# ymartin101/RTS

Measured on AMD Instinct MI355X. Metric: Mrays/s (primary+bounces) & ms/pulse, 100k-tri scene, higher is better.
Workload: dtype f64

## Files before the change

### rts_amd/csrc/rts_api.hip

```cpp
#include <cmath>
#include <cstdarg>
#include <cstdio>
#include <cstring>
#include <cstdlib>
#include <dlfcn.h>
#include <algorithm>
#include <chrono>
#include <map>
#include <memory>
#include <mutex>
#include <stdexcept>
#include <string>
#include <thread>
#include "rts_internal.h"
#include "rts_raygen.h"
#include <atomic>

static thread_local char g_err[1024] = "";
void rts_set_error(const char* fmt, ...) { va_list ap; va_start(ap, fmt); vsnprintf(g_err, sizeof(g_err), fmt, ap); va_end(ap); }
extern "C" const char* rts_last_error(void) { return g_err; }
#include "rts_build_id.h"
extern "C" const char* rts_build_id(void) { return RTS_SOURCE_HASH; }

#include <dirent.h>
#include <sched.h>
extern "C" int rts_bind_host_to_device(int device, int* numa_node)
{
    if (numa_node) *numa_node = -1;
    char bdf[64] = {0};
    if (hipDeviceGetPCIBusId(bdf, (int)sizeof(bdf), device) != hipSuccess) { (void)hipGetLastError(); rts_set_error("rts_bind_host_to_device: no PCI address for device %d", device); return RTS_ERR_INVALID; }
    for (char* q = bdf; *q; q++) *q = (char)tolower((unsigned char)*q);
    char path[256]; snprintf(path, sizeof(path), "/sys/bus/pci/devices/%s/numa_node", bdf);
    int node = -1;
    if (FILE* f = fopen(path, "r")) { if (fscanf(f, "%d", &node) != 1) node = -1; fclose(f); }
    if (node < 0) return RTS_OK;
    snprintf(path, sizeof(path), "/sys/devices/system/node/node%d/cpulist", node);
    cpu_set_t want; CPU_ZERO(&want); int n_want = 0;
    if (FILE* f = fopen(path, "r")) {
        int a = 0, b = 0; char sep = 0;
        while (fscanf(f, "%d", &a) == 1) {
            b = a;
            int ch = fgetc(f);
            if (ch == '-') { if (fscanf(f, "%d", &b) != 1) b = a; ch = fgetc(f); }
            for (int k = a; k <= b && k < CPU_SETSIZE; k++) { CPU_SET(k, &want); n_want++; }
            sep = (char)ch; if (sep != ',') break;
        }
        fclose(f);
    }
    if (n_want == 0) return RTS_OK;
    cpu_set_t have; CPU_ZERO(&have);
    if (sched_getaffinity(0, sizeof(have), &have) != 0) return RTS_OK;
    cpu_set_t both; CPU_AND(&both, &want, &have);
    if (CPU_COUNT(&both) == 0) return RTS_OK;
    if (DIR* d = opendir("/proc/self/task")) {
        while (struct dirent* e = readdir(d)) { const int tid = atoi(e->d_name); if (tid > 0) (void)sched_setaffinity(tid, sizeof(both), &both); }
        closedir(d);
    } else (void)sched_setaffinity(0, sizeof(both), &both);
    if (numa_node) *numa_node = node;
    return RTS_OK;
}

extern int rts_fill_i32(hipStream_t st, int32_t* p, int32_t v, size_t n);

__global__ void k_children_to_prims(RtsNode4* __restrict__ nodes, uint32_t n, const uint32_t* __restrict__ leaf_prim)
{
    const uint32_t i = blockIdx.x * blockDim.x + threadIdx.x;
    if (i >= n) return;
    for (int k = 0; k < 4; k++) { const int32_t ch = nodes[i].child[k]; nodes[i].pad[k] = ch; if (ch < 0) nodes[i].child[k] = ~(int32_t)leaf_prim[~ch]; }
}

__global__ void k_node_versions(const RtsNode4* __restrict__ nodes, uint32_t n, RtsNode4* __restrict__ out, int key_mode)
{
    const uint32_t g = blockIdx.x * blockDim.x + threadIdx.x;
    if (g >= n * 8u) return;
    const uint32_t i = g >> 3, o = g & 7u;
    const RtsNode4 nd = nodes[i];
    const bool mx = (o & 1u) != 0u, my = (o & 2u) != 0u, mz = (o & 4u) != 0u;
    float key[4]; int ord[4];
    for (int k = 0; k < 4; k++) {
        const float ex = mx ? -nd.hix[k] : nd.lox[k], ey = my ? -nd.hiy[k] : nd.loy[k], ez = mz ? -nd.hiz[k] : nd.loz[k];
        const float cx = 0.5f * (nd.lox[k] + nd.hix[k]), cy = 0.5f * (nd.loy[k] + nd.hiy[k]), cz = 0.5f * (nd.loz[k] + nd.hiz[k]);
        const float kc = key_mode == 1 ? ((mx ? -cx : cx) + (my ? -cy : cy) + (mz ? -cz : cz)) : (ex + ey + ez);
        key[k] = nd.child[k] == 0x7fffffff ? __builtin_inff() : kc;
        ord[k] = k;
    }
    for (int a = 1; a < 4; a++)
        for (int b = a; b > 0 && key[ord[b]] < key[ord[b - 1]]; b--) { const int t = ord[b]; ord[b] = ord[b - 1]; ord[b - 1] = t; }
    RtsNode4 v;
    for (int j = 0; j < 4; j++) {
        const int k = ord[j];
        v.lox[j] = mx ? nd.hix[k] : nd.lox[k]; v.hix[j] = mx ? nd.lox[k] : nd.hix[k];
        v.loy[j] = my ? nd.hiy[k] : nd.loy[k]; v.hiy[j] = my ? nd.loy[k] : nd.hiy[k];
        v.loz[j] = mz ? nd.hiz[k] : nd.loz[k]; v.hiz[j] = mz ? nd.loz[k] : nd.hiz[k];
        const int32_t ch = nd.child[k];
        v.child[j] = (ch >= 0 && ch != 0x7fffffff) ? (int32_t)(((uint32_t)ch << 3) | o) : ch;
        v.pad[j] = nd.pad[k];
    }
    out[g] = v;
// ... 157 lines not shown
        const RtsMesh& m = meshes[t];
        if ((m.n_triangles && !m.triangles) || (m.n_vertices && !m.vertices) || (m.n_normals && !m.normals)) { rts_set_error("rts_set_scene: target %u has null arrays", t); return RTS_ERR_INVALID; }
        mh[t].n_tris = m.n_triangles; mh[t].n_verts = m.n_vertices; mh[t].n_normals = m.n_normals;
        mh[t].tri_base = (uint32_t)nt; mh[t].vert_base = (uint32_t)nv; mh[t].normal_base = (uint32_t)nn;
        mh[t].refl_coeff = m.refl_coeff; mh[t].refr_index = m.refr_index;
        mh[t].perface = m.n_normals > m.n_vertices;
        nt += m.n_triangles; nv += m.n_vertices; nn += m.n_normals;
        if (nt > 0x7ffffff0ULL || nv > 0x7ffffff0ULL || nn > 0x7ffffff0ULL) { rts_set_error("rts_set_scene: scene too large"); return RTS_ERR_UNSUPPORTED; }
    }
    std::vector<uint32_t> vidx(3*nt), nidx(3*nt), vtarg(nv), ntarg(nn), ptarg(nt);
    std::vector<double> verts(3*nv), normals(3*nn);
    for (uint32_t t = 0; t < n_targets; t++) {
        const RtsMesh& m = meshes[t]; const RtsMeshHost& h = mh[t];
        for (uint32_t i = 0; i < m.n_triangles; i++) {
            for (int k = 0; k < 3; k++) {
                uint32_t v = m.triangles[3*(size_t)i + k];
                if (v >= m.n_vertices) { rts_set_error("rts_set_scene: target %u triangle %u references vertex %u >= %u", t, i, v, m.n_vertices); return RTS_ERR_INVALID; }
                vidx[3*((size_t)h.tri_base + i) + k] = h.vert_base + v;
                uint32_t ni = h.perface ? i : v;
                if (m.n_normals == 0) ni = 0; else if (ni >= m.n_normals) { rts_set_error("rts_set_scene: target %u normal index %u >= %u", t, ni, m.n_normals); return RTS_ERR_INVALID; }
                nidx[3*((size_t)h.tri_base + i) + k] = h.normal_base + ni;
            }
            ptarg[(size_t)h.tri_base + i] = t;
        }
        if (m.n_triangles && m.n_normals == 0 && c->params.interpolate_smooth) { rts_set_error("rts_set_scene: target %u has no normals but interpolate_smooth is set", t); return RTS_ERR_INVALID; }
        for (uint32_t i = 0; i < m.n_vertices; i++) { vtarg[(size_t)h.vert_base + i] = t; for (int k = 0; k < 3; k++) verts[3*((size_t)h.vert_base + i) + k] = m.vertices[3*(size_t)i + k]; }
        for (uint32_t i = 0; i < m.n_normals; i++) { ntarg[(size_t)h.normal_base + i] = t; for (int k = 0; k < 3; k++) normals[3*((size_t)h.normal_base + i) + k] = m.normals[3*(size_t)i + k]; }
    }
    std::unique_ptr<RtsScene> guard(new RtsScene());
    RtsScene* ns = guard.get(); ns->device = c->device;
    RTS_HIP(hipStreamSynchronize(c->stream));
    RTS_HIP(ns->d_tri_vidx.reserve(3*nt + 1)); RTS_HIP(ns->d_tri_nidx.reserve(3*nt + 1)); RTS_HIP(ns->d_vert_targ.reserve(nv + 1)); RTS_HIP(ns->d_norm_targ.reserve(nn + 1));
    RTS_HIP(ns->d_prim_targ.reserve(nt + 1)); RTS_HIP(ns->d_verts_local.reserve(3*nv + 1)); RTS_HIP(ns->d_normals_local.reserve(3*nn + 1));
    if (nt) { RTS_HIP(hipMemcpy(ns->d_tri_vidx.p, vidx.data(), sizeof(uint32_t)*3*nt, hipMemcpyHostToDevice)); RTS_HIP(hipMemcpy(ns->d_tri_nidx.p, nidx.data(), sizeof(uint32_t)*3*nt, hipMemcpyHostToDevice));
              RTS_HIP(hipMemcpy(ns->d_prim_targ.p, ptarg.data(), sizeof(uint32_t)*nt, hipMemcpyHostToDevice)); }
    if (nv) { RTS_HIP(hipMemcpy(ns->d_vert_targ.p, vtarg.data(), sizeof(uint32_t)*nv, hipMemcpyHostToDevice)); RTS_HIP(hipMemcpy(ns->d_verts_local.p, verts.data(), sizeof(double)*3*nv, hipMemcpyHostToDevice)); }
    if (nn) { RTS_HIP(hipMemcpy(ns->d_norm_targ.p, ntarg.data(), sizeof(uint32_t)*nn, hipMemcpyHostToDevice)); RTS_HIP(hipMemcpy(ns->d_normals_local.p, normals.data(), sizeof(double)*3*nn, hipMemcpyHostToDevice)); }
    ns->meshes = mh; ns->n_prims = (uint32_t)nt; ns->n_verts = (uint32_t)nv; ns->n_normals = (uint32_t)nn;

    const auto t_build0 = std::chrono::steady_clock::now();
    RtsSceneTuning st; st.device_build = (c->params.flags & RTS_FLAG_HOST_BUILD) == 0;
    rts_tuning_read(&st, rts_env);
    bool device_build = st.device_build;
    const double split_budget = st.split_budget;
    if (device_build) {
        int rc = rts_lbvh_build_device(c, ns, vidx, mh, st);
        if (rc == RTS_OK && st.fail_device_build) { rts_set_error("rts_set_scene: device builder failure injected (RTS_DEBUG_FAIL_DEVICE_BUILD)"); rc = RTS_ERR_HIP; }
        if (rc != RTS_OK) {
            if (rc == RTS_ERR_INVALID || !st.build_fallback) return rc;
            (void)hipGetLastError();
            fprintf(stderr, "[rts] device hierarchy build failed (%s): falling back to the host builder\n", rts_last_error());
            ns->d_nodes4.release(); ns->d_leaf_prim.release(); ns->blas.clear(); ns->n_nodes = 0; ns->n_leaves = 0;
            device_build = false;
        } else ns->builder = 1;
    }
    if (!device_build) {
        std::vector<RtsNode4> nodes4; std::vector<uint32_t> leaf_prim; std::vector<RtsBlasInfo> blas(n_targets);
        {
            std::vector<std::vector<RtsNode4>> pn(n_targets); std::vector<std::vector<uint32_t>> pl(n_targets); std::vector<int> prc(n_targets, RTS_OK);
            for (uint32_t t0 = 0; t0 < n_targets; t0 += 16) {
                std::vector<std::thread> pool;
                for (uint32_t t = t0; t < std::min(n_targets, t0 + 16); t++)
                    pool.emplace_back([&, t]() { prc[t] = rts_sah_build(meshes[t].vertices, meshes[t].triangles, meshes[t].n_triangles, split_budget, pn[t], pl[t], blas[t]); });
                for (auto& th : pool) th.join();
            }
            for (uint32_t t = 0; t < n_targets; t++) {
                if (prc[t] != RTS_OK) return prc[t];
                const int32_t node_base = (int32_t)nodes4.size(), leaf_base = (int32_t)leaf_prim.size();
                for (RtsNode4 nd : pn[t]) {
                    for (int k = 0; k < 4; k++) { int32_t& ch = nd.child[k]; if (ch == 0x7fffffff) continue; if (ch >= 0) ch += node_base; else ch = ~(~ch + leaf_base); }
                    nodes4.push_back(nd);
                }
                for (uint32_t lp : pl[t]) leaf_prim.push_back(lp + mh[t].tri_base);
                if (blas[t].root >= 0) blas[t].root += node_base;
            }
        }
        RTS_HIP(ns->d_nodes4.reserve(nodes4.size() + 1)); RTS_HIP(ns->d_leaf_prim.reserve(leaf_prim.size() + 1));
        if (!nodes4.empty()) RTS_HIP(hipMemcpy(ns->d_nodes4.p, nodes4.data(), sizeof(RtsNode4)*nodes4.size(), hipMemcpyHostToDevice));
        if (!leaf_prim.empty()) RTS_HIP(hipMemcpy(ns->d_leaf_prim.p, leaf_prim.data(), sizeof(uint32_t)*leaf_prim.size(), hipMemcpyHostToDevice));
        ns->blas = blas; ns->n_nodes = (uint32_t)nodes4.size(); ns->n_leaves = (uint32_t)leaf_prim.size();
        ns->builder = 0;
    }
    if (ns->n_nodes) { k_children_to_prims<<<(ns->n_nodes + 255) / 256, 256, 0, c->stream>>>(ns->d_nodes4.p, ns->n_nodes, ns->d_leaf_prim.p); RTS_HIP(hipGetLastError()); RTS_HIP(hipStreamSynchronize(c->stream)); }
    {
        const bool want = st.node_versions;
        const int key_mode = st.version_key_centre ? 1 : 0;
        size_t free_b = 0, total_b = 0; (void)hipMemGetInfo(&free_b, &total_b);
        const size_t need = (size_t)ns->n_nodes * 8 * sizeof(RtsNode4);
        if (want && ns->n_nodes && ns->n_nodes < (1u << 28) && need < free_b / 4) {
            if (ns->d_nodes4v.reserve((size_t)ns->n_nodes * 8) == hipSuccess) {
                k_node_versions<<<(ns->n_nodes * 8u + 255u) / 256u, 256, 0, c->stream>>>(ns->d_nodes4.p, ns->n_nodes, ns->d_nodes4v.p, key_mode);
                RTS_HIP(hipGetLastError()); RTS_HIP(hipStreamSynchronize(c->stream));
            } else (void)hipGetLastError();
        }
    }
    ns->build_ms = std::chrono::duration<double, std::milli>(std::chrono::steady_clock::now() - t_build0).count();

    rts_scene_unref(c->scene);
    c->scene = guard.release();
    return rts_attach_scene(c);
}

static int rts_attach_scene(RtsContext* c)
{
    const RtsScene* sc = c->scene; const uint32_t n_targets = (uint32_t)sc->meshes.size();
    RTS_HIP(c->d_leaves.reserve((size_t)sc->n_prims + 1));
    RTS_HIP(c->d_verts_world.reserve(3*(size_t)sc->n_verts + 1)); RTS_HIP(c->d_normals_world.reserve(3*(size_t)sc->n_normals + 1));
    {
        const size_t span = offsetof(RtsPinned, cnt);
        RTS_HIP(c->d_params.reserve(span));
        c->p_lc = reinterpret_cast<RtsLaunchConsts*>(c->d_params.p + offsetof(RtsPinned, lc));
        c->p_motion = reinterpret_cast<RtsTargetMotion*>(c->d_params.p + offsetof(RtsPinned, motion));
        c->p_targets = reinterpret_cast<RtsTargetDev*>(c->d_params.p + offsetof(RtsPinned, td));
        c->rcs_uploaded = false;
    }
    c->verts_world_valid = false; c->order_sum_valid = false;
    if (c->hist->refs.load() > 1) { rts_hist_unref(c->hist); c->hist = new RtsTileHist(); }
    c->motion.assign(n_targets, RtsTargetMotion{}); c->motion_valid = false; c->bvh_valid = false; c->hist->n = 0; c->hist->any = false; c->hist->head_hint_valid = false; c->tile_cost_pending = false; c->tile_last_valid = false;
    return RTS_OK;
}

extern "C" int rts_share_scene(RtsHandle dst, RtsHandle src)
{
    if (!dst || !src || dst == src) { rts_set_error("rts_share_scene: needs two distinct handles"); return RTS_ERR_INVALID; }
    if (dst->device != src->device) { rts_set_error("rts_share_scene: handles live on different devices (%d, %d)", dst->device, src->device); return RTS_ERR_INVALID; }
    if (dst->params.interpolate_smooth && !src->params.interpolate_smooth) {
        for (const RtsMeshHost& m : src->scene->meshes) if (m.n_tris && m.n_normals == 0) { rts_set_error("rts_share_scene: the scene has a mesh without normals but the receiving handle interpolates normals"); return RTS_ERR_INVALID; }
    }
    RtsContext* c = dst;
    CHECK_HANDLE(c);
    CHECK_CLOSED(c);
    RTS_HIP(hipStreamSynchronize(c->stream));
    if (dst->scene == src->scene) return RTS_OK;
    rts_scene_unref(dst->scene);
    dst->scene = src->scene; dst->scene->refs++;
    { int rc = rts_attach_scene(dst); if (rc != RTS_OK) return rc; }
    if (dst->tune.share_history && src->tune.share_history && dst->params.width == src->params.width) {
        rts_hist_unref(dst->hist);
        dst->hist = src->hist; dst->hist->refs++;
    }
    return RTS_OK;
}

extern "C" int rts_scene_info(RtsHandle c, RtsSceneInfo* out)
{
    if (!c || !out) { rts_set_error("rts_scene_info: null argument"); return RTS_ERR_INVALID; }
    const RtsScene* sc = c->scene;
    memset(out, 0, sizeof(*out));
    out->n_targets = (uint32_t)sc->meshes.size(); out->n_prims = sc->n_prims; out->n_nodes = sc->n_nodes; out->n_leaves = sc->n_leaves;
    out->handles_sharing = (uint32_t)sc->refs.load(); out->builder = sc->builder; out->build_ms = sc->build_ms;
    out->shared_device_bytes = sc->device_bytes(); out->version_bytes = sc->d_nodes4v.cap * sizeof(RtsNode4);
    out->handle_device_bytes = c->d_leaves.cap * sizeof(RtsLeafTri) + c->d_verts_world.cap * 8 + c->d_normals_world.cap * 8 + c->d_params.cap;
    return RTS_OK;
}

extern "C" int rts_set_receivers(RtsHandle c, const RtsReceiverSphere* rx, uint32_t n_rx)
{
    CHECK_HANDLE(c);
    CHECK_CLOSED(c);
    if (n_rx && !rx) { rts_set_error("rts_set_receivers: null array"); return RTS_ERR_INVALID; }
    if (n_rx > 65535) { rts_set_error("rts_set_receivers: more than 65535 receivers"); return RTS_ERR_UNSUPPORTED; }
    { int rc = check_key_width(c->depth, (uint32_t)c->scene->meshes.size(), n_rx, "rts_set_receivers"); if (rc != RTS_OK) return rc; }
    std::vector<RtsRxDev> h(n_rx);
    for (uint32_t i = 0; i < n_rx; i++) {
        const RtsReceiverSphere& r = rx[i];
        const double vals[8] = { r.centre[0], r.centre[1], r.centre[2], r.radius, r.min_theta, r.max_theta, r.min_phi, r.max_phi };
// ... 1164 lines not shown
```

### rts_amd/csrc/rts_bvh.hip

```cpp
#include <cstring>
#include <hip/hip_runtime.h>
#include "rts_internal.h"
#include "rts_ray_ops.h"

__device__ __forceinline__ void place_one(const double* __restrict__ local, double* __restrict__ world, const uint32_t* __restrict__ targ_of,
                                          const RtsTargetMotion* __restrict__ motion, uint32_t i, bool add_position)
{
    const RtsTargetMotion m = motion[targ_of[i]];
    double x = local[3*i], y = local[3*i+1], z = local[3*i+2];
    if (m.has_rotation) {
        double rx = 0.0, ry = 0.0, rz = 0.0;
        rx += m.rotation[0] * x; rx += m.rotation[1] * y; rx += m.rotation[2] * z;
        ry += m.rotation[3] * x; ry += m.rotation[4] * y; ry += m.rotation[5] * z;
        rz += m.rotation[6] * x; rz += m.rotation[7] * y; rz += m.rotation[8] * z;
        x = rx; y = ry; z = rz;
    }
    if (add_position) { x += m.position[0]; y += m.position[1]; z += m.position[2]; }
    world[3*i] = x; world[3*i+1] = y; world[3*i+2] = z;
}
__global__ void k_place(const double* __restrict__ v_local, double* __restrict__ v_world, const uint32_t* __restrict__ v_targ, uint32_t n_verts,
                        const double* __restrict__ n_local, double* __restrict__ n_world, const uint32_t* __restrict__ n_targ, uint32_t n_normals,
                        const RtsTargetMotion* __restrict__ motion)
{
    const uint32_t i = blockIdx.x * blockDim.x + threadIdx.x;
    if (i < n_verts) place_one(v_local, v_world, v_targ, motion, i, true);
    else if (i - n_verts < n_normals) place_one(n_local, n_world, n_targ, motion, i - n_verts, false);
}

#define RTS_MASK_TILE_WORDS 2048
struct RtsMaskLds { uint32_t tile[RTS_MASK_TILE_WORDS]; int box[4]; };
__device__ __forceinline__ void rts_mask_mark(RtsMaskLds& S, const bool have, const double (&p)[9], const double ox, const double oy, const double oz, const RtsMaskFrame& f, uint32_t* __restrict__ mask)
{
    uint32_t* flag = mask + (size_t)f.n * f.n / 32u;
    if (threadIdx.x == 0) { S.box[0] = 0x7fffffff; S.box[1] = 0x7fffffff; S.box[2] = -1; S.box[3] = -1; }
    __syncthreads();
    int iu0 = 0, iu1 = -1, iv0 = 0, iv1 = -1;
    if (have) {
        double u[3], v[3]; bool finite = true, front = true;
        for (int k = 0; k < 3; k++) {
            const double px = p[3*k] - ox, py = p[3*k + 1] - oy, pz = p[3*k + 2] - oz;
            finite = finite && isfinite(px) && isfinite(py) && isfinite(pz);
            const double w = px * (double)f.bx + py * (double)f.by + pz * (double)f.bz;
            front = front && (w > 0.0) && (w * w > 1.0e-6 * (px*px + py*py + pz*pz));
            u[k] = (px * (double)f.ux + py * (double)f.uy + pz * (double)f.uz) / w;
            v[k] = (px * (double)f.vx + py * (double)f.vy + pz * (double)f.vz) / w;
        }
        if (finite && !front) atomicExch(flag, 1u);
        if (finite && front) {
            const double fu0 = (fmin(fmin(u[0], u[1]), u[2]) - (double)f.u0) * (double)f.inv_du, fu1 = (fmax(fmax(u[0], u[1]), u[2]) - (double)f.u0) * (double)f.inv_du;
            const double fv0 = (fmin(fmin(v[0], v[1]), v[2]) - (double)f.v0) * (double)f.inv_dv, fv1 = (fmax(fmax(v[0], v[1]), v[2]) - (double)f.v0) * (double)f.inv_dv;
            const double nn = (double)f.n;
            if (!(fu1 < -1.0 || fv1 < -1.0 || fu0 > nn || fv0 > nn)) {
                iu0 = (int)fmax(floor(fu0) - 1.0, 0.0); iu1 = (int)fmin(floor(fu1) + 1.0, nn - 1.0);
                iv0 = (int)fmax(floor(fv0) - 1.0, 0.0); iv1 = (int)fmin(floor(fv1) + 1.0, nn - 1.0);
                if ((long long)(iu1 - iu0 + 1) * (long long)(iv1 - iv0 + 1) > RTS_MASK_MAX_CELLS) { atomicExch(flag, 1u); iu1 = iu0 - 1; }
            }
        }
    }
    const bool any = iu1 >= iu0 && iv1 >= iv0;
    if (any) { atomicMin(&S.box[0], iu0); atomicMin(&S.box[1], iv0); atomicMax(&S.box[2], iu1); atomicMax(&S.box[3], iv1); }
    __syncthreads();
    if (S.box[2] < 0) return;
    const int W0 = S.box[0] >> 5, V0 = S.box[1], TW = (S.box[2] >> 5) - W0 + 1, TH = S.box[3] - V0 + 1;
    const bool tiled = (long long)TW * TH <= RTS_MASK_TILE_WORDS;
    if (tiled) { for (int w = threadIdx.x; w < TW * TH; w += blockDim.x) S.tile[w] = 0u; __syncthreads(); }
    if (any) {
        for (int iv = iv0; iv <= iv1; iv++) {
            for (int w0 = iu0 >> 5; w0 <= (iu1 >> 5); w0++) {
                const int lo = max(iu0, w0 << 5) & 31, hi = min(iu1, (w0 << 5) + 31) & 31;
                const uint32_t bits = (hi == 31 ? 0xffffffffu : ((1u << (hi + 1)) - 1u)) & ~((1u << lo) - 1u);
                if (tiled) atomicOr(&S.tile[(iv - V0) * TW + (w0 - W0)], bits);
                else atomicOr(&mask[((size_t)iv * f.n >> 5) + (size_t)w0], bits);
            }
        }
    }
    if (!tiled) return;
    __syncthreads();
    for (int w = threadIdx.x; w < TW * TH; w += blockDim.x) {
        const uint32_t bits = S.tile[w];
        if (bits) atomicOr(&mask[((size_t)(V0 + w / TW) * f.n >> 5) + (size_t)(W0 + w % TW)], bits);
    }
}

__device__ __forceinline__ void place_vertex(const double* __restrict__ local, const RtsTargetMotion& m, uint32_t i, double* __restrict__ out3)
{
    double x = local[3*(size_t)i], y = local[3*(size_t)i+1], z = local[3*(size_t)i+2];
    if (m.has_rotation) {
        double rx = 0.0, ry = 0.0, rz = 0.0;
        rx += m.rotation[0] * x; rx += m.rotation[1] * y; rx += m.rotation[2] * z;
        ry += m.rotation[3] * x; ry += m.rotation[4] * y; ry += m.rotation[5] * z;
        rz += m.rotation[6] * x; rz += m.rotation[7] * y; rz += m.rotation[8] * z;
        x = rx; y = ry; z = rz;
    }
    x += m.position[0]; y += m.position[1]; z += m.position[2];
    out3[0] = x; out3[1] = y; out3[2] = z;
}
template <bool LEAVES, bool MASK, bool PLACE = false>
__global__ void __launch_bounds__(256) k_leaves(const uint32_t* __restrict__ leaf_prim, const uint32_t* __restrict__ tri_vidx, const double* __restrict__ verts,
                                                const uint32_t* __restrict__ prim_targ, RtsLeafTri* __restrict__ leaves, uint32_t n,
                                                double ox, double oy, double oz, RtsMaskFrame f, uint32_t* __restrict__ mask,
                                                const RtsTargetMotion* __restrict__ motion = nullptr, uint32_t prim_blocks = 0, const double* __restrict__ n_local = nullptr,
                                                double* __restrict__ n_world = nullptr, const uint32_t* __restrict__ n_targ = nullptr, uint32_t n_normals = 0)
{
    __shared__ __attribute__((aligned(16))) uint32_t s_raw[MASK ? sizeof(RtsMaskLds) / 4 : 1];
    if (PLACE && blockIdx.x >= prim_blocks) {
        const uint32_t q = (blockIdx.x - prim_blocks) * blockDim.x + threadIdx.x;
        if (q < n_normals) place_one(n_local, n_world, n_targ, motion, q, false);
        return;
    }
    const uint32_t i = blockIdx.x * blockDim.x + threadIdx.x;
    double p[9] = {0, 0, 0, 0, 0, 0, 0, 0, 0};
    if (i < n) {
        const uint32_t g = leaf_prim ? leaf_prim[i] : i;
        const uint32_t a = tri_vidx[3*(size_t)g], b = tri_vidx[3*(size_t)g+1], c = tri_vidx[3*(size_t)g+2];
        if (PLACE) {
            const RtsTargetMotion m = motion[prim_targ[g]];
            place_vertex(verts, m, a, p); place_vertex(verts, m, b, p + 3); place_vertex(verts, m, c, p + 6);
        } else {
        p[0] = verts[3*(size_t)a]; p[1] = verts[3*(size_t)a+1]; p[2] = verts[3*(size_t)a+2];
        p[3] = verts[3*(size_t)b]; p[4] = verts[3*(size_t)b+1]; p[5] = verts[3*(size_t)b+2];
        p[6] = verts[3*(size_t)c]; p[7] = verts[3*(size_t)c+1]; p[8] = verts[3*(size_t)c+2];
        }
        if (LEAVES) {
            dvec3 e0, e1, nn;
            tri_terms(mk3(p[0], p[1], p[2]), mk3(p[3], p[4], p[5]), mk3(p[6], p[7], p[8]), e0, e1, nn);
            RtsLeafTri L;
            L.p0x = p[0]; L.p0y = p[1]; L.p0z = p[2]; L.e0x = e0.x; L.e0y = e0.y; L.e0z = e0.z; L.e1x = e1.x; L.e1y = e1.y; L.e1z = e1.z;
            L.nx = nn.x; L.ny = nn.y; L.nz = nn.z;
            L.prim = g; L.targ = prim_targ[g]; L.pad[0] = 0u; L.pad[1] = 0u;
            leaves[i] = L;
        }
    }
    if (MASK) rts_mask_mark(*reinterpret_cast<RtsMaskLds*>(s_raw), i < n, p, ox, oy, oz, f, mask);
}

static inline unsigned blocks_for(size_t n, unsigned bs) { return (unsigned)((n + bs - 1) / bs); }

int rts_scene_place(RtsContext* c, const RtsLaunchConsts& lc, bool place, uint32_t* pmask)
{
    hipStream_t st = c->stream;
    const RtsMaskFrame& f = lc.mask;
    const bool mask = f.n != 0;
    const RtsScene* sc = c->scene;
    if (place && sc->n_prims) {
        const unsigned gp = blocks_for(sc->n_prims, 256), gn = blocks_for(sc->n_normals, 256);
        if (mask) k_leaves<true, true, true><<<gp + gn, 256, 0, st>>>(nullptr, sc->d_tri_vidx.p, sc->d_verts_local.p, sc->d_prim_targ.p, c->d_leaves.p, sc->n_prims, lc.ox, lc.oy, lc.oz, f, pmask,
                                                                     c->p_motion, gp, sc->d_normals_local.p, c->d_normals_world.p, sc->d_norm_targ.p, sc->n_normals);
        else k_leaves<true, false, true><<<gp + gn, 256, 0, st>>>(nullptr, sc->d_tri_vidx.p, sc->d_verts_local.p, sc->d_prim_targ.p, c->d_leaves.p, sc->n_prims, lc.ox, lc.oy, lc.oz, f, nullptr,
                                                                  c->p_motion, gp, sc->d_normals_local.p, c->d_normals_world.p, sc->d_norm_targ.p, sc->n_normals);
        c->verts_world_valid = false;
        RTS_HIP(hipGetLastError());
        return RTS_OK;
    }
    if (place) {
        if (sc->n_verts + sc->n_normals) k_place<<<blocks_for((size_t)sc->n_verts + sc->n_normals, 256), 256, 0, st>>>(sc->d_verts_local.p, c->d_verts_world.p, sc->d_vert_targ.p, sc->n_verts,
                                                                                                                         sc->d_normals_local.p, c->d_normals_world.p, sc->d_norm_targ.p, sc->n_normals, c->p_motion);
        c->verts_world_valid = true;
    } else if (mask) {
        if (!c->verts_world_valid && sc->n_verts) {
            k_place<<<blocks_for((size_t)sc->n_verts, 256), 256, 0, st>>>(sc->d_verts_local.p, c->d_verts_world.p, sc->d_vert_targ.p, sc->n_verts, sc->d_normals_local.p, c->d_normals_world.p, sc->d_norm_targ.p, 0u, c->p_motion);
            c->verts_world_valid = true;
        }
        if (sc->n_prims) k_leaves<false, true><<<blocks_for(sc->n_prims, 256), 256, 0, st>>>(nullptr, sc->d_tri_vidx.p, c->d_verts_world.p, sc->d_prim_targ.p, nullptr, sc->n_prims, lc.ox, lc.oy, lc.oz, f, pmask);
    }
    RTS_HIP(hipGetLastError());
    return RTS_OK;
}
```

### rts_amd/csrc/rts_internal.h

```cpp
#pragma once
#include <hip/hip_runtime.h>
#include <stdint.h>
#include <stddef.h>
#include <atomic>
#include <string>
#include <vector>
#include "../../include/rts_amd.h"
#include "rts_device_math.h"
#include "rts_pattern.h"
#include "rts_waveform.h"
#include "rts_noise.h"
#include "rts_image.h"
#include "rts_cube_source.h"
#include "rts_stft.h"
#include "rts_beat.h"
#include "rts_beam.h"
#include "rts_adapt.h"
#include "rts_cfar_os.h"
#include "rts_owned.h"
#include "rts_launch_plan.h"
#include "rts_post_plan.h"
#include "rts_pulse_state.h"
#include "rts_tuning.h"
static_assert(RtsTuning().img_split_below == RTS_IMAGE_SPLIT_BELOW, "the default of RTS_IMAGE_SPLIT_BELOW is rts_image.h's");
// ... 88 lines not shown
    double w1x, w1y, w1z;
    uint64_t ray_first;
    uint32_t W, pad;
    uint32_t w_magic, w_more;
    uint32_t il_tile, il_parts, il_part, pad2;
    const uint32_t* il_list;
    RtsMaskFrame mask;
    float f_bs[3], f_st[3], f_m[9], f_pad;
};
static_assert(sizeof(RtsLaunchConsts) % 8 == 0, "launch constants are copied to LDS dword by dword");

struct RtsTraceArgs {
    const RtsLaunchConsts* lc;
    uint64_t ray_first;
    uint32_t n_rays, W;
    uint32_t max_refl, smooth;
    uint32_t n_prims, n_targets, n_rx, keep_all;
    uint32_t max_refr, rows;
    RtsChildState* child;
    const RtsNode4* nodes4;
    const RtsNode4* nodes4v;
    const RtsLeafTri* leaves;
    const uint32_t* tri_nidx;
    const double* normals;
    const RtsTargetDev* targets;
    const RtsRxDev* rx;
    RtsEndRecord* recv_records;
    RtsEndRecord* all_records;
    unsigned long long* counters;
    unsigned long long* block_counters;
    float* dir_hist;
    int32_t* hit_prim;
    float* hit_t;
    int32_t* stack_ovf;
    uint32_t total_threads;
    uint32_t slab_threads;
    const uint32_t* tile_order;
    uint32_t* tile_cost;
    uint32_t* tile_ctr;
    uint32_t coop_spread;
    const uint32_t* tile_head;
    const uint32_t* tile_head_all;
    const uint32_t* tile_live;
    uint32_t rx_window_screen;
    uint32_t coop_versions;
    uint32_t batch_dead;
    uint32_t coop_walk_steps_lo;
    uint32_t coop_min_cost, coop_walk_steps;
    unsigned long long* timeline;
    uint32_t pre_filter;
    const uint32_t* pmask;
    uint32_t stack_lds;
};

struct RtsMeshHost {
    uint32_t n_tris, n_verts, n_normals;
    uint32_t tri_base, vert_base, normal_base;
    double refl_coeff, refr_index;
    bool perface;
};

#define RTS_PIN_GROUPS 4096
static inline uint32_t rts_agg_spec(uint32_t R) { return R < RTS_PIN_GROUPS ? R : RTS_PIN_GROUPS; }
struct RtsPinned {
    RtsLaunchConsts lc;
    RtsTargetMotion motion[256];
    RtsTargetDev td[256];
    unsigned long long cnt[16];
    uint32_t G, pad;
    double rcs[256];
    double gsum[5 * RTS_PIN_GROUPS]; uint64_t gkey[RTS_PIN_GROUPS]; uint64_t grow[RTS_PIN_GROUPS]; uint32_t gmin[RTS_PIN_GROUPS];
};

struct RtsGate { hipStream_t tstream = nullptr; std::atomic<int> refs{0}; int device = 0; };

struct RtsScene {
    std::atomic<int> refs{1}; int device = 0;
    std::vector<RtsMeshHost> meshes;
    uint32_t n_prims = 0, n_verts = 0, n_normals = 0;
    DevBuf<uint32_t> d_tri_vidx, d_tri_nidx, d_vert_targ, d_norm_targ, d_prim_targ;
    DevBuf<double> d_verts_local, d_normals_local;
    std::vector<RtsBlasInfo> blas; uint32_t n_nodes = 0, n_leaves = 0;
    DevBuf<RtsNode4> d_nodes4; DevBuf<uint32_t> d_leaf_prim;
    DevBuf<RtsNode4> d_nodes4v;
    double build_ms = 0; uint32_t builder = 0;
    size_t device_bytes() const {
        return d_tri_vidx.cap * 4 + d_tri_nidx.cap * 4 + d_vert_targ.cap * 4 + d_norm_targ.cap * 4 + d_prim_targ.cap * 4 + d_verts_local.cap * 8 +
               d_normals_local.cap * 8 + (d_nodes4.cap + d_nodes4v.cap) * sizeof(RtsNode4) + d_leaf_prim.cap * 4;
    }
};

struct RtsTileHist { std::atomic<int> refs{1}; DevBuf<uint32_t> d; uint32_t n = 0; bool any = false; uint32_t head_hint = 0; bool head_hint_valid = false; };

struct RtsSpecParams { std::vector<double> rcs; double wl = 0, gt = 0, gr = 0, carrier = 0, cspeed = 0; int32_t cube_pulse = -1; uint64_t base = 0;
                       int mode = 0;
                       int fin = 0;
                       std::vector<double> pat_rx; double pat_org[3] = {0, 0, 0}, pat_dir[2] = {0, 0};
};
struct RtsPatArgs { const RtsPatView* pats; const double* rx; uint32_t n_rx, n_targets; double ox, oy, oz, tx_az, tx_el, wl, carrier, cspeed; };
struct RtsHostMirror {
    PinBuf<char> buf; uint32_t cap = 0, D = 0;
    size_t o_rays = 0, o_paths = 0, o_angles = 0, o_slots = 0, o_apower = 0, o_adoppler = 0, o_adelay = 0, o_aphase = 0, o_apm = 0, o_vpower = 0, o_vdoppler = 0;
    bool recv_valid = false, agg_valid = false;
    bool want = false;
};
struct RtsAggPending { bool valid = false, rows = false; uint32_t R = 0, D = 0, spec = 0; RtsKeyPlan key = {}; uint64_t base = 0; double* gsum = nullptr; };

struct RtsCubeProduct {
    DevBuf<double> own; double* p = nullptr; size_t doubles = 0; bool valid = false;
    hipError_t place(void* device_out, size_t n, double** out)
    {
        *out = (double*)device_out; if (*out) return hipSuccess;
        if (n > own.cap) { p = nullptr; doubles = 0; valid = false; }
        const hipError_t e = own.reserve(n); *out = own.p; return e;
    }
    void record(double* out, size_t n) { p = out; doubles = n; valid = true; }
};

struct RtsCubeState {
    RtsCubeParams params = {}; double* p = nullptr; DevBuf<double> own; bool set = false;
    DevBuf<double> d_wave; uint32_t wave_M = 0, wave_L = 0; bool wave_set = false;
    RtsCubeProduct doppler; uint32_t doppler_n = 0;
    DevBuf<uint32_t> d_det_cnt, d_det_off; DevBuf<uint8_t> d_det_tmp; DevBuf<RtsDetection> d_det; uint32_t det_nseg = 0, det_max = 0; bool det_valid = false;
    StagedUpload<double> os_alpha; std::vector<double> os_tab; uint32_t os_tab_key[5] = {0, 0, 0, 0, 0}; double os_tab_pfa = 0.0; bool os_tab_sent = false;
    RtsCubeProduct image; uint32_t img_nx = 0, img_ny = 0;
    StagedUpload<double> img_geo; DevBuf<double> d_img_scratch;
    RtsCubeProduct stft;
    StagedUpload<double> stft_win; DevBuf<double> d_stft_part;
    DevBuf<double> d_beat_part;
    RtsCubeProduct range;
    StagedUpload<double> range_win;
    RtsCubeProduct beam;
    StagedUpload<double> beam_w;
    RtsCubeProduct cov; uint32_t cov_n = 0; DevBuf<double> d_cov_part;
    RtsCubeProduct mvdr;
    StagedUpload<double> mvdr_s; DevBuf<uint32_t> d_mvdr_status;
    void end_products() { doppler.valid = false; det_valid = false; image.valid = false; stft.valid = false; range.valid = false; beam.valid = false; cov.valid = false; mvdr.valid = false; }
};

struct RtsPulseResults {
    uint64_t n_recv = 0;
    const unsigned long long* recv_dev = nullptr;
    std::vector<RtsGroup> groups; bool agg_valid = false; uint64_t recv_index_base = 0;
    RtsAggPending agg_pending;
    bool agg_delay_in = true;
    int64_t agg_base_local = 0;
    RtsHostMirror mirror;
    std::vector<PerRayData> v_rays; std::vector<int32_t> v_paths; std::vector<double> v_angles, v_apower, v_adoppler, v_adelay, v_aphase; std::vector<uint64_t> v_slots; std::vector<int32_t> v_apm;
    std::vector<PerRayData> v_agg_rays; unsigned v_recv_have = 0;
    bool agg_timed = false, fin_timed = false;
    void forget() { agg_valid = false; agg_pending.valid = false; n_recv = 0; mirror.want = false; mirror.recv_valid = false; mirror.agg_valid = false; v_recv_have = 0; }
};
#define RTS_DEV_COUNT(R_dev, R, beyond) do { if (R_dev) { const unsigned long long v_ = *(R_dev); if (v_ > (unsigned long long)(R)) { beyond; } else (R) = (uint32_t)v_; } } while (0)

struct RtsContext {
    RtsParams params;
    RtsTuning tune;
    uint32_t depth = 0;
    int device = 0;
    hipStream_t stream = nullptr;
    hipStream_t tstream = nullptr;
    hipStream_t cstream = nullptr; hipEvent_t ev_coop[2] = {nullptr, nullptr};
    uint32_t n_head_hint = 0;
    uint32_t last_coop_grid = 0;
    hipEvent_t ev[9] = {nullptr, nullptr, nullptr, nullptr, nullptr, nullptr, nullptr, nullptr, nullptr};
    RtsScene* scene = nullptr;
    DevBuf<double> d_verts_world, d_normals_world;
    std::vector<RtsTargetMotion> motion; bool motion_valid = false; bool bvh_valid = false;
    DevBuf<char> d_params;
    RtsLaunchConsts* p_lc = nullptr; RtsTargetMotion* p_motion = nullptr; RtsTargetDev* p_targets = nullptr;
    DevBuf<RtsLeafTri> d_leaves; DevBuf<char> d_sort_tmp;
// ... 113 lines not shown
```

Baseline: 24070.

## Order primitives by BVH leaf order for spatially coherent mask marking, band the LDS tile

At scene build, a permutation of primitives is computed in BVH leaf order and uploaded. k_leaves then processes triangles in that order, so each block's triangles are spatially close. This shrinks the per-block bounding box in the mask frame, letting more blocks use the LDS tile instead of global atomics. The mask marking also reduces the box with a warp shuffle before touching LDS atomics, and replaces the global-atomic fallback with bands of rows that each fit the tile. The cost is a one-time host round trip at build plus scattered leaf writes (leaves[g]).

```diff
diff --git a/rts_amd/csrc/rts_api.hip b/rts_amd/csrc/rts_api.hip
--- a/rts_amd/csrc/rts_api.hip
+++ b/rts_amd/csrc/rts_api.hip
@@ -14,6 +14,7 @@
 #include <thread>
 #include "rts_internal.h"
 #include "rts_raygen.h"
+#include "rts_prim_order.h"
 #include <atomic>
 
 static thread_local char g_err[1024] = "";
@@ -337,6 +338,14 @@
         ns->builder = 0;
     }
     if (ns->n_nodes) { k_children_to_prims<<<(ns->n_nodes + 255) / 256, 256, 0, c->stream>>>(ns->d_nodes4.p, ns->n_nodes, ns->d_leaf_prim.p); RTS_HIP(hipGetLastError()); RTS_HIP(hipStreamSynchronize(c->stream)); }
+    if (ns->n_prims) {
+        std::vector<uint32_t> slots(ns->n_leaves);
+        RTS_HIP(hipStreamSynchronize(c->stream));
+        if (ns->n_leaves) RTS_HIP(hipMemcpy(slots.data(), ns->d_leaf_prim.p, sizeof(uint32_t) * ns->n_leaves, hipMemcpyDeviceToHost));
+        const std::vector<uint32_t> order = rts_prim_order(slots.data(), slots.size(), ns->n_prims);
+        RTS_HIP(ns->d_prim_order.reserve(order.size() + 1));
+        RTS_HIP(hipMemcpy(ns->d_prim_order.p, order.data(), sizeof(uint32_t) * order.size(), hipMemcpyHostToDevice));
+    }
     {
         const bool want = st.node_versions;
         const int key_mode = st.version_key_centre ? 1 : 0;
diff --git a/rts_amd/csrc/rts_bvh.hip b/rts_amd/csrc/rts_bvh.hip
--- a/rts_amd/csrc/rts_bvh.hip
+++ b/rts_amd/csrc/rts_bvh.hip
@@ -28,6 +28,7 @@
 }
 
 #define RTS_MASK_TILE_WORDS 2048
+static_assert(RTS_MASK_N / 32u <= RTS_MASK_TILE_WORDS, "a band of the mask tile holds at least one whole row");
 struct RtsMaskLds { uint32_t tile[RTS_MASK_TILE_WORDS]; int box[4]; };
 __device__ __forceinline__ void rts_mask_mark(RtsMaskLds& S, const bool have, const double (&p)[9], const double ox, const double oy, const double oz, const RtsMaskFrame& f, uint32_t* __restrict__ mask)
 {
@@ -58,27 +59,36 @@
         }
     }
     const bool any = iu1 >= iu0 && iv1 >= iv0;
-    if (any) { atomicMin(&S.box[0], iu0); atomicMin(&S.box[1], iv0); atomicMax(&S.box[2], iu1); atomicMax(&S.box[3], iv1); }
+    {
+        int b0 = any ? iu0 : 0x7fffffff, b1 = any ? iv0 : 0x7fffffff, b2 = any ? iu1 : -1, b3 = any ? iv1 : -1;
+        for (int d = warpSize / 2; d > 0; d >>= 1) {
+            b0 = min(b0, __shfl_xor(b0, d)); b1 = min(b1, __shfl_xor(b1, d)); b2 = max(b2, __shfl_xor(b2, d)); b3 = max(b3, __shfl_xor(b3, d));
+        }
+        if ((threadIdx.x & (warpSize - 1)) == 0 && b2 >= 0) { atomicMin(&S.box[0], b0); atomicMin(&S.box[1], b1); atomicMax(&S.box[2], b2); atomicMax(&S.box[3], b3); }
+    }
     __syncthreads();
     if (S.box[2] < 0) return;
     const int W0 = S.box[0] >> 5, V0 = S.box[1], TW = (S.box[2] >> 5) - W0 + 1, TH = S.box[3] - V0 + 1;
-    const bool tiled = (long long)TW * TH <= RTS_MASK_TILE_WORDS;
-    if (tiled) { for (int w = threadIdx.x; w < TW * TH; w += blockDim.x) S.tile[w] = 0u; __syncthreads(); }
-    if (any) {
-        for (int iv = iv0; iv <= iv1; iv++) {
-            for (int w0 = iu0 >> 5; w0 <= (iu1 >> 5); w0++) {
-                const int lo = max(iu0, w0 << 5) & 31, hi = min(iu1, (w0 << 5) + 31) & 31;
-                const uint32_t bits = (hi == 31 ? 0xffffffffu : ((1u << (hi + 1)) - 1u)) & ~((1u << lo) - 1u);
-                if (tiled) atomicOr(&S.tile[(iv - V0) * TW + (w0 - W0)], bits);
-                else atomicOr(&mask[((size_t)iv * f.n >> 5) + (size_t)w0], bits);
+    const int band = RTS_MASK_TILE_WORDS / TW;
+    for (int b0 = 0; b0 < TH; b0 += band) {
+        const int B0 = V0 + b0, bh = min(band, TH - b0), nw = TW * bh;
+        if (b0) __syncthreads();
+        for (int w = threadIdx.x; w < nw; w += blockDim.x) S.tile[w] = 0u;
+        __syncthreads();
+        if (any) {
+            for (int iv = max(iv0, B0); iv <= min(iv1, B0 + bh - 1); iv++) {
+                for (int w0 = iu0 >> 5; w0 <= (iu1 >> 5); w0++) {
+                    const int lo = max(iu0, w0 << 5) & 31, hi = min(iu1, (w0 << 5) + 31) & 31;
+                    const uint32_t bits = (hi == 31 ? 0xffffffffu : ((1u << (hi + 1)) - 1u)) & ~((1u << lo) - 1u);
+                    atomicOr(&S.tile[(iv - B0) * TW + (w0 - W0)], bits);
+                }
             }
         }
-    }
-    if (!tiled) return;
-    __syncthreads();
-    for (int w = threadIdx.x; w < TW * TH; w += blockDim.x) {
-        const uint32_t bits = S.tile[w];
-        if (bits) atomicOr(&mask[((size_t)(V0 + w / TW) * f.n >> 5) + (size_t)(W0 + w % TW)], bits);
+        __syncthreads();
+        for (int w = threadIdx.x; w < nw; w += blockDim.x) {
+            const uint32_t bits = S.tile[w];
+            if (bits) atomicOr(&mask[((size_t)(B0 + w / TW) * f.n >> 5) + (size_t)(W0 + w % TW)], bits);
+        }
     }
 }
 
@@ -96,7 +106,7 @@
     out3[0] = x; out3[1] = y; out3[2] = z;
 }
 template <bool LEAVES, bool MASK, bool PLACE = false>
-__global__ void __launch_bounds__(256) k_leaves(const uint32_t* __restrict__ leaf_prim, const uint32_t* __restrict__ tri_vidx, const double* __restrict__ verts,
+__global__ void __launch_bounds__(256) k_leaves(const uint32_t* __restrict__ order, const uint32_t* __restrict__ tri_vidx, const double* __restrict__ verts,
                                                 const uint32_t* __restrict__ prim_targ, RtsLeafTri* __restrict__ leaves, uint32_t n,
                                                 double ox, double oy, double oz, RtsMaskFrame f, uint32_t* __restrict__ mask,
                                                 const RtsTargetMotion* __restrict__ motion = nullptr, uint32_t prim_blocks = 0, const double* __restrict__ n_local = nullptr,
@@ -111,7 +121,7 @@
     const uint32_t i = blockIdx.x * blockDim.x + threadIdx.x;
     double p[9] = {0, 0, 0, 0, 0, 0, 0, 0, 0};
     if (i < n) {
-        const uint32_t g = leaf_prim ? leaf_prim[i] : i;
+        const uint32_t g = order[i];
         const uint32_t a = tri_vidx[3*(size_t)g], b = tri_vidx[3*(size_t)g+1], c = tri_vidx[3*(size_t)g+2];
         if (PLACE) {
             const RtsTargetMotion m = motion[prim_targ[g]];
@@ -128,7 +138,7 @@
             L.p0x = p[0]; L.p0y = p[1]; L.p0z = p[2]; L.e0x = e0.x; L.e0y = e0.y; L.e0z = e0.z; L.e1x = e1.x; L.e1y = e1.y; L.e1z = e1.z;
             L.nx = nn.x; L.ny = nn.y; L.nz = nn.z;
             L.prim = g; L.targ = prim_targ[g]; L.pad[0] = 0u; L.pad[1] = 0u;
-            leaves[i] = L;
+            leaves[g] = L;
         }
     }
     if (MASK) rts_mask_mark(*reinterpret_cast<RtsMaskLds*>(s_raw), i < n, p, ox, oy, oz, f, mask);
@@ -144,9 +154,9 @@
     const RtsScene* sc = c->scene;
     if (place && sc->n_prims) {
         const unsigned gp = blocks_for(sc->n_prims, 256), gn = blocks_for(sc->n_normals, 256);
-        if (mask) k_leaves<true, true, true><<<gp + gn, 256, 0, st>>>(nullptr, sc->d_tri_vidx.p, sc->d_verts_local.p, sc->d_prim_targ.p, c->d_leaves.p, sc->n_prims, lc.ox, lc.oy, lc.oz, f, pmask,
+        if (mask) k_leaves<true, true, true><<<gp + gn, 256, 0, st>>>(sc->d_prim_order.p, sc->d_tri_vidx.p, sc->d_verts_local.p, sc->d_prim_targ.p, c->d_leaves.p, sc->n_prims, lc.ox, lc.oy, lc.oz, f, pmask,
                                                                      c->p_motion, gp, sc->d_normals_local.p, c->d_normals_world.p, sc->d_norm_targ.p, sc->n_normals);
-        else k_leaves<true, false, true><<<gp + gn, 256, 0, st>>>(nullptr, sc->d_tri_vidx.p, sc->d_verts_local.p, sc->d_prim_targ.p, c->d_leaves.p, sc->n_prims, lc.ox, lc.oy, lc.oz, f, nullptr,
+        else k_leaves<true, false, true><<<gp + gn, 256, 0, st>>>(sc->d_prim_order.p, sc->d_tri_vidx.p, sc->d_verts_local.p, sc->d_prim_targ.p, c->d_leaves.p, sc->n_prims, lc.ox, lc.oy, lc.oz, f, nullptr,
                                                                   c->p_motion, gp, sc->d_normals_local.p, c->d_normals_world.p, sc->d_norm_targ.p, sc->n_normals);
         c->verts_world_valid = false;
         RTS_HIP(hipGetLastError());
@@ -161,7 +171,7 @@
             k_place<<<blocks_for((size_t)sc->n_verts, 256), 256, 0, st>>>(sc->d_verts_local.p, c->d_verts_world.p, sc->d_vert_targ.p, sc->n_verts, sc->d_normals_local.p, c->d_normals_world.p, sc->d_norm_targ.p, 0u, c->p_motion);
             c->verts_world_valid = true;
         }
-        if (sc->n_prims) k_leaves<false, true><<<blocks_for(sc->n_prims, 256), 256, 0, st>>>(nullptr, sc->d_tri_vidx.p, c->d_verts_world.p, sc->d_prim_targ.p, nullptr, sc->n_prims, lc.ox, lc.oy, lc.oz, f, pmask);
+        if (sc->n_prims) k_leaves<false, true><<<blocks_for(sc->n_prims, 256), 256, 0, st>>>(sc->d_prim_order.p, sc->d_tri_vidx.p, c->d_verts_world.p, sc->d_prim_targ.p, nullptr, sc->n_prims, lc.ox, lc.oy, lc.oz, f, pmask);
     }
     RTS_HIP(hipGetLastError());
     return RTS_OK;
diff --git a/rts_amd/csrc/rts_internal.h b/rts_amd/csrc/rts_internal.h
--- a/rts_amd/csrc/rts_internal.h
+++ b/rts_amd/csrc/rts_internal.h
@@ -194,11 +194,12 @@
     DevBuf<double> d_verts_local, d_normals_local;
     std::vector<RtsBlasInfo> blas; uint32_t n_nodes = 0, n_leaves = 0;
     DevBuf<RtsNode4> d_nodes4; DevBuf<uint32_t> d_leaf_prim;
+    DevBuf<uint32_t> d_prim_order;
     DevBuf<RtsNode4> d_nodes4v;
     double build_ms = 0; uint32_t builder = 0;
     size_t device_bytes() const {
         return d_tri_vidx.cap * 4 + d_tri_nidx.cap * 4 + d_vert_targ.cap * 4 + d_norm_targ.cap * 4 + d_prim_targ.cap * 4 + d_verts_local.cap * 8 +
-               d_normals_local.cap * 8 + (d_nodes4.cap + d_nodes4v.cap) * sizeof(RtsNode4) + d_leaf_prim.cap * 4;
+               d_normals_local.cap * 8 + (d_nodes4.cap + d_nodes4v.cap) * sizeof(RtsNode4) + d_leaf_prim.cap * 4 + d_prim_order.cap * 4;
     }
 };
 
diff --git a/rts_amd/csrc/rts_prim_order.h b/rts_amd/csrc/rts_prim_order.h
--- /dev/null
+++ b/rts_amd/csrc/rts_prim_order.h
@@ -0,0 +1,16 @@
+#pragma once
+#include <cstddef>
+#include <cstdint>
+#include <vector>
+
+static inline std::vector<uint32_t> rts_prim_order(const uint32_t* leaf_prim, size_t n_leaves, uint32_t n_prims)
+{
+    std::vector<uint32_t> order; order.reserve(n_prims);
+    std::vector<uint8_t> seen(n_prims, 0);
+    for (size_t s = 0; s < n_leaves; s++) {
+        const uint32_t g = leaf_prim[s];
+        if (g < n_prims && !seen[g]) { seen[g] = 1; order.push_back(g); }
+    }
+    for (uint32_t g = 0; g < n_prims; g++) if (!seen[g]) order.push_back(g);
+    return order;
+}
```

Measured after the change: 24680, median of 6. 2.5% higher.
